# ERGO-Code/HiGHS

Hardware: AMD Instinct MI355X
Metric: PDHG iterations/sec (higher is better)
Workload: dtype f64; 1 GPU; synthetic random sparse LP 1Mx1M, 8M nnz (seed 1); m=1000000, n=1000000, nnz=7999977, parallelism=single GPU, options=presolve=off, kkt_tolerance=1e-4, adaptive step + restarts (reference defaults)

## Files before the change

### highs_amd/csrc/pdlp_halpern.cpp

```cpp
#include "pdlp_halpern.hpp"
#include "pdlp_halpernfn.hpp"

#include <algorithm>
#include <climits>
#include <cmath>
#include <cstdarg>
#include <cstdio>
#include <cstdlib>
#include <cstring>
#include <limits>

namespace pdlp {

namespace {
constexpr int kCheckInterval = 40;
constexpr int kStatSlots = 8;
constexpr int kSlotFpe = kHSlotFpe, kSlotCheck = kHSlotCheck, kSlotFpe0 = kHSlotFpe0, kSlotDiff = kHSlotDiff, kStatOut = kHStatOut;
static_assert(kSlotFpe0 == kSlotCheck + kHRowStats + kHColStats && kSlotDiff == kSlotFpe0 + 3 && kSlotDiff + 2 <= kStatOut, "stat slots");
}

double HalpernSolver::elapsed() const {
  return std::chrono::duration<double>(std::chrono::steady_clock::now() - solveBeg_).count();
}

// ... 683 lines not shown
    runBlock(false);
    enqueueFpe(kSlotFpe, nullptr);
    fetchStats(3);
    hostState_->fpe = halpernFpe(*hostState_, hostStats_ + kSlotFpe);
    put(0, hostState_->fpe);
  } else if (name == "steps") {
    const int k = out && cap > 0 ? (int)out[0] : kCheckInterval;
    if (k < 1 || k > kCheckInterval) throw std::runtime_error("steps: 1..40");
    armState();
    pushState();
    for (int i = 1; i <= k; ++i) enqueueStep(i == 1 || i == k, i);
  } else if (name == "mesh_phases") {
    double us[3] = {0, 0, 0}, cnt[3] = {0, 0, 0};
    if (mesh_) mesh_->phaseStats(us, cnt, stream_);
    for (int k = 0; k < 3; ++k) { put(k, us[k]); put(3 + k, cnt[k]); }
  } else if (name == "exchange") {
    put(0, sharded_ ? 2.0 : 0.0);
  } else if (name == "profile_on" || name == "profile_off") {
    profile_ = name == "profile_on";
  } else {
    throw std::runtime_error("unknown stage: " + name);
  }
  PDLP_HIP(hipStreamSynchronize(stream_));
}

double HalpernSolver::timeKernel(const std::string& name, int32_t reps) {
  if (reps < 1) reps = 1;
  armState();
  pushState();
  const HalpernVecs h = stepVecs(false, 2);
// ... 23 lines not shown
```

### highs_amd/csrc/pdlp_kernels.hip

```cpp
#include "pdlp_kernels.hpp"

#include <type_traits>

#include <algorithm>
#include <climits>
#include <cmath>
#include <cstddef>

#include "pdlp_checkfn.hpp"
#include "pdlp_devfn.hpp"

namespace pdlp {

namespace {

enum Epilogue { kPlain = 0, kDualStep = 1, kAtyInteract = 2, kAtyPartial = 3, kHalpernPrimal = 4, kHalpernDual = 5, kAtyFused = 6,
                kQxInteract = 7 };
constexpr bool usesDevState(int epi) {
  return epi == kDualStep || epi == kAtyInteract || epi == kAtyPartial || epi == kAtyFused || epi == kQxInteract;
}
constexpr bool isInteract(int epi) { return epi == kAtyInteract || epi == kAtyFused; }

struct SpmvArgs {
  SpmvMat A;
// ... 278 lines not shown
    }
    __syncthreads();
    for (int r = rFirst; r < r1; r += kSpmvThreads) {
      if (r != rFirst) {
        qb = a.A.beg[r] - p0;
        qe = a.A.beg[r + 1] - p0;
        pre = epi.prefetch(vecIndex(r));
      }
      const double s = majorSum(prod, qb, qe);
      epi.apply(vecIndex(r), s, pre);
    }
    epi.template finish<kSpmvThreads>(a.A.partOffset + blk, scratch);
  }
}

constexpr int kSlabSlots = 3;
template <int EPI, bool TWO, bool CC = false, bool ULO = false>
__global__ __launch_bounds__(kSlabThreads, TWO ? 2 * kSlabThreads / 256 : kSlabThreads / 256) void k_spmv_slab(const SpmvArgs a) {
  constexpr int NB = kSlabSlots;
  constexpr int GD = 1;
  constexpr bool LATE = EPI == kAtyFused && !TWO;
  if (EPI == kAtyFused && a.st->halted) {
    if (blockIdx.x == 0 && threadIdx.x < sizeof(DevState) / 4)
      reinterpret_cast<uint32_t*>(a.stOut)[threadIdx.x] = reinterpret_cast<const uint32_t*>(a.st)[threadIdx.x];
    return;
  }
  if (usesDevState(EPI) && a.st->halted) return;
  if ((EPI == kHalpernPrimal || EPI == kHalpernDual) && a.h.hs->halted) return;
  if (EPI == kPlain && !gateOpen(a.gate)) return;
  static_assert(GD >= 1 && NB >= GD + 2, "entry loads need two steps, gathers GD steps");
  const unsigned long long tProf0 = a.prof ? wall_clock64() : 0ull;
  int profBlk = (int)blockIdx.x;
// ... 80 lines not shown
      }
      for (; j < end; ++j) s += stg[j];
      wacc[lrow] = s;
    };
    if (descs == 0) {
      if (isHead) addRun();
    } else {
      const int seg = (int)__builtin_amdgcn_mbcnt_hi((uint32_t)(descs >> 32), __builtin_amdgcn_mbcnt_lo((uint32_t)descs, 0u)) + (desc ? 1 : 0);
      const int nSeg = __popcll(descs) + 1;
      for (int sg = 0; sg < nSeg; ++sg) {
        if (isHead && seg == sg) addRun();
        __builtin_amdgcn_wave_barrier();
      }
    }
  };
  const uint32_t* __restrict__ ent = a.S.ent + e0;
  const double* __restrict__ val = a.S.val + e0;
  const int cnt = e1 - e0;
  const int nG = (cnt + kWave - 1) / kWave;
  const int last = cnt > 0 ? cnt - 1 : 0;
  auto entryIndex = [&](int g) { const int q = g * kWave + lane; return q < last ? q : last; };
  auto gather = [&](uint32_t e) -> double {
    const uint32_t off = (e & mmask) << 3;
    return *reinterpret_cast<const double*>(reinterpret_cast<const char*>(in) + off);
  };
  uint32_t E[NB];
  double V[NB], X[NB];
#pragma unroll
  for (int k = 0; k < NB; ++k) {
    if (k + GD >= NB) X[(k + GD) % NB] = gather(E[(k + GD) % NB]);
    const int q = entryIndex(k);
    E[k] = ent[q];
    V[k] = val[q];
    __builtin_amdgcn_sched_barrier(0);
  }
  int nRounds = (nG + NB - 1) / NB;
  {
    int* share = reinterpret_cast<int*>(scratch);
    if (lane == 0) share[wave] = nRounds;
    __syncthreads();
#pragma unroll
    for (int w = 0; w < kWaves; ++w) nRounds = share[w] > nRounds ? share[w] : nRounds;
    __syncthreads();
  }
  for (int o = 0; o < nRounds; ++o) {
#pragma unroll
    for (int u = 0; u < NB; ++u) {
      const int g = o * NB + u;
      X[(u + GD) % NB] = gather(E[(u + GD) % NB]);
      const int nValid = cnt - g * kWave;
      const uint32_t eCur = E[u];
      const double prod = V[u] * X[u];
      {
        const int q = entryIndex(g + NB);
        E[u] = ent[q];
        V[u] = val[q];
      }
      __builtin_amdgcn_sched_barrier(0);
      consumeGroup(eCur, prod, nValid);
      if (!a.S.noPace) __syncthreads();
    }
  }
  if (a.S.noPace) __syncthreads();

  profStamp(0);
  const uint32_t* __restrict__ mask = a.S.longMask;
  auto longMajor = [&](int r) { return ((mask[r >> 5] >> (r & 31)) & 1u) != 0u; };
#pragma unroll
  for (int k = 0; k < kSlabPre; ++k) {
    const int lr = tid + k * kSlabThreads;
    if (rBase + lr < rEnd && !longMajor(rBase + lr)) epi.apply(rBase + lr, acc[lr], pre[k]);
  }
  for (int lr0 = tid + kSlabPre * kSlabThreads; rBase + lr0 < rEnd; lr0 += kSlabPre * kSlabThreads) {
    Pre more[kSlabPre];
#pragma unroll
    for (int k = 0; k < kSlabPre; ++k) {
      const int r = rBase + lr0 + k * kSlabThreads;
      more[k] = epi.prefetch(r < rEnd ? r : rEnd - 1);
// ... 495 lines not shown
    }
    return p;
  }();
  return prof;
}

template <int EPI>
void launchSpmv(const MatView& M, SpmvArgs a, hipStream_t s) {
  a.xcdMap = M.xcdMap;
  if (EPI == kDualStep && M.useSlab && M.slab.nBlocks <= 512) a.prof = slabProf();
  a.L = M.lng;
  a.A = M.csr;
  const int nTasks = M.lng.nTasks;
  if (M.useSlab && M.slab.nBlocks > 0) {
    a.S = M.slab;
    const size_t lds = (size_t)((M.slab.rowsPerBlock + 1) & ~1) * 8 + kSlabThreads * 8 + 2 * (kSlabThreads / kWave) * 8;
    const dim3 grid(M.slab.nBlocks + (nTasks + M.lng.taskGroup - 1) / M.lng.taskGroup);
    if (nTasks > 0) hipLaunchKernelGGL((k_spmv_slab<EPI, true>), grid, dim3(kSlabThreads), lds, s, a);
    else hipLaunchKernelGGL((k_spmv_slab<EPI, false>), grid, dim3(kSlabThreads), lds, s, a);
  } else if (M.csr.nBlocks > 0 || nTasks > 0) {
    const dim3 grid(M.csr.nBlocks + (nTasks + kSpmvThreads / kWave - 1) / (kSpmvThreads / kWave)), block(kSpmvThreads);
    if (M.csr.chunk == kChunkSmall) hipLaunchKernelGGL((k_spmv<EPI, kChunkSmall>), grid, block, 0, s, a);
    else hipLaunchKernelGGL((k_spmv<EPI, kChunk>), grid, block, 0, s, a);
  }
  if (nTasks > 0 && M.lng.contrib && (EPI == kDualStep || EPI == kAtyInteract || EPI == kQxInteract))
    hipLaunchKernelGGL(k_long_groups, dim3((M.lng.nSlots + kVecThreads - 1) / kVecThreads), dim3(kVecThreads), 0, s, M.lng,
                       a.st, a.part0, EPI == kAtyInteract ? a.part1 : nullptr);
}
}

void launchSpmvAxDual(const MatView& A, const IterVecs& v, const DevState* st, double* partDY, hipStream_t s) {
  SpmvArgs a{};
  a.st = st; a.v = v; a.part0 = partDY;
  launchSpmv<kDualStep>(A, a, s);
}
void launchSpmvAtyInteract(const MatView& At, const IterVecs& v, const DevState* st, double* partDX,
                           double* partInter, hipStream_t s) {
  SpmvArgs a{};
  a.st = st; a.v = v; a.part0 = partDX; a.part1 = partInter;
  launchSpmv<kAtyInteract>(At, a, s);
}
namespace {
size_t fusedLds(const MatView& At) {
  return (size_t)((At.slab.rowsPerBlock + 1) & ~1) * 8 + kSlabThreads * 8 + 2 * (kSlabThreads / kWave) * 8 + 4 * (kVecThreads / kWave) * 8 +
         sizeof(DevState) + 16;
}
}
namespace {
int fusedTaskGroups(const MatView& At) { return (At.lng.nTasks + At.lng.taskGroup - 1) / At.lng.taskGroup; }
}
int fusedCoTaskBlocks(const MatView& At, int device) {
  if (!At.useSlab || At.lng.nTasks <= 0 || At.lng.contrib != nullptr || At.slab.nBlocks <= 0) return 0;
  int perCu = 0, cus = 0;
  if (hipOccupancyMaxActiveBlocksPerMultiprocessor(&perCu, k_spmv_slab<kAtyFused, true>, kSlabThreads, fusedLds(At)) != hipSuccess) return 0;
  if (hipDeviceGetAttribute(&cus, hipDeviceAttributeMultiprocessorCount, device) != hipSuccess) return 0;
  const int groups = fusedTaskGroups(At);
  if (perCu < 2 || At.slab.nBlocks > cus || groups > cus) return 0;
  return groups;
}
int fusedAtyBlocksResident(const MatView& At, int device) {
  (void)slabProf();
  if (!At.useSlab || At.slab.nBlocks <= 0 || (At.lng.nTasks > 0 && At.lng.contrib != nullptr)) return 0;
  int perCu = 0, cus = 0;
  const hipError_t e = At.coTaskBlocks > 0
                           ? hipOccupancyMaxActiveBlocksPerMultiprocessor(&perCu, k_spmv_slab<kAtyFused, true>, kSlabThreads, fusedLds(At))
                           : hipOccupancyMaxActiveBlocksPerMultiprocessor(&perCu, k_spmv_slab<kAtyFused, false>, kSlabThreads, fusedLds(At));
  if (e != hipSuccess) return 0;
  if (hipDeviceGetAttribute(&cus, hipDeviceAttributeMultiprocessorCount, device) != hipSuccess) return 0;
  return perCu * cus;
}
int fusedAtyBlocks(const MatView& At) { return At.slab.nBlocks + At.coTaskBlocks; }
void launchSpmvAtyFusedPrimal(const MatView& At, const IterVecs& v, const DevState* stIn, DevState* stOut,
                              const double* partDY, int32_t nDY, double* partDX, double* partInter, unsigned long long* bar,
                              hipStream_t s, int32_t timeoutMs, int32_t faultTrial) {
  SpmvArgs a{};
  a.barLimit = (unsigned long long)(timeoutMs > 0 ? timeoutMs : 1000) * 100000ull;
  a.faultTrial = faultTrial;
  a.coTaskBlocks = At.lng.nTasks > 0 ? At.coTaskBlocks : 0;
  a.inlineTasks = At.lng.nTasks > 0 && a.coTaskBlocks == 0 ? 1 : 0;
  a.touchTail = At.touchTail;
  a.st = stIn; a.v = v; a.part0 = partDX; a.part1 = partInter;
  a.stOut = stOut; a.partDY = partDY; a.nDY = nDY; a.nDX = At.nPartials; a.bar = bar;
  if (At.slab.nBlocks <= 512) a.prof = slabProf();
  a.xcdMap = At.xcdMap; a.L = At.lng; a.A = At.csr; a.S = At.slab;
  const dim3 gridTwo(At.slab.nBlocks + a.coTaskBlocks), gridOne(At.slab.nBlocks), block(kSlabThreads);
  const size_t lds = fusedLds(At);
  auto launchTwo = [&](auto cc, auto ulo) {
    hipLaunchKernelGGL((k_spmv_slab<kAtyFused, true, decltype(cc)::value, decltype(ulo)::value>), gridTwo, block, lds, s, a);
  };
  auto launchOne = [&](auto cc, auto ulo) {
    hipLaunchKernelGGL((k_spmv_slab<kAtyFused, false, decltype(cc)::value, decltype(ulo)::value>), gridOne, block, lds, s, a);
  };
  auto pick = [&](auto&& launch) {
    using T = std::true_type; using F = std::false_type;
    if (v.constCached) { if (v.lowerUniform) launch(T{}, T{}); else launch(T{}, F{}); }
    else { if (v.lowerUniform) launch(F{}, T{}); else launch(F{}, F{}); }
  };
  if (a.coTaskBlocks > 0) pick(launchTwo);
  else pick(launchOne);
}
void launchSpmvAtyPartial(const MatView& At, const IterVecs& v, const DevState* st, double* out, hipStream_t s) {
  SpmvArgs a{};
  a.st = st; a.v = v; a.out = out;
  launchSpmv<kAtyPartial>(At, a, s);
}
void launchHalpernPrimal(const MatView& At, const HalpernVecs& h, hipStream_t s) {
// ... 184 lines not shown
```

### highs_amd/csrc/pdlp_kernels.hpp

```cpp
#pragma once
#include <hip/hip_runtime.h>

#include <cstdint>

#include "pdlp_env.hpp"

namespace pdlp {

constexpr int kChunk = 2048;
constexpr int kChunkSmall = 512;
constexpr int64_t kChunkSmallBelowNnz = 1 << 18;
inline int32_t spmvChunkFor(int64_t nnz) { return nnz < kChunkSmallBelowNnz ? kChunkSmall : kChunk; }
constexpr int kSpmvThreads = 256;
constexpr int kMaxMajorsPerBlock = 2048;
constexpr int kVecThreads = 256;

struct DevState {
  double eta;
  double beta;
  double tau, sigma;
  double primalStep, dualStep;
  double sumPrimalStep, sumDualStep;
  double avgW;
  double avgWx;
// ... 79 lines not shown
  int32_t nSlots;
  int32_t groupSize;
  int32_t taskGroup;
};

constexpr int kSlabThreads = 1024;
constexpr int kSlabMaxRows = 16384;
struct SlabMat {
  const int32_t* wavePtr;
  const uint32_t* ent;
  const double* val;
  const uint32_t* longMask;
  const int32_t* waveBeg;
  int32_t nMajor, nBlocks, rowsPerBlock, minorBits;
  int32_t noPace;
};
constexpr int kSlabTileLog2 = 14;

struct MatView {
  SpmvMat csr;
  SlabMat slab;
  LongMat lng;
  int32_t useSlab;
  int32_t nPartials;
  int32_t xcdMap;
  int32_t coTaskBlocks;
  int32_t touchTail;
};

struct IterVecs {
  double* x[2];
// ... 205 lines not shown
```

### highs_amd/csrc/pdlp_setup.hip

```cpp
#include "pdlp_setup.hpp"

#include <cstring>

#include <rocprim/rocprim.hpp>

#include <algorithm>
#include <cmath>
#include <limits>

namespace pdlp {

namespace {

constexpr int kT = 256;
inline int gridFor(int64_t n) { return (int)std::max<int64_t>(1, std::min<int64_t>((n + kT - 1) / kT, 65535 * 16)); }
#define GSTRIDE(i, n) for (int64_t i = (int64_t)blockIdx.x * blockDim.x + threadIdx.x; i < (n); i += (int64_t)gridDim.x * blockDim.x)

constexpr double kBoundInf = 1e20;

__device__ __forceinline__ bool isEqKind(int k) { return k == kRowEq || k == kRowBound || k == kRowFree; }
__global__ void k_row_classify(const double* __restrict__ lo, const double* __restrict__ up, int m, double infThresh,
                               int freeKind, int32_t* kind, int32_t* eqFlag, int32_t* ineqFlag, int32_t* slackFlag) {
  GSTRIDE(i, m) {
    const bool hl = lo[i] > -infThresh, hu = up[i] < infThresh;
// ... 677 lines not shown
  sortByKey(keys.get(), nnz, (uint64_t)keyMax, sortedKeys, perm, s);
  L.wavePtr.alloc((size_t)nWaves + 1);
  hipLaunchKernelGGL(k_wave_ptr, dim3(gridFor(nWaves + 1)), dim3(kT), 0, s, sortedKeys.get(), nnz, nWaves, S,
                     L.wavePtr.get());
  L.nnzShort = fetchOne(L.wavePtr.get() + nWaves, s);
  L.ent.alloc((size_t)L.nnzShort + 1);
  L.val.alloc((size_t)L.nnzShort + 1);
  L.ent.zero(s);
  L.val.zero(s);
  if (L.nnzShort > 0)
    hipLaunchKernelGGL(k_slab_entries, dim3(gridFor(L.nnzShort)), dim3(kT), 0, s, perm.get(), M.major.get(),
                       M.idx.get(), M.val.get(), L.nnzShort, waveOf.get(), L.waveBeg.get(), L.minorBits, L.ent.get(), L.val.get());
  PDLP_HIP(hipStreamSynchronize(s));
}

}
```

### highs_amd/csrc/pdlp_setup.hpp

```cpp
#pragma once
#include <hip/hip_runtime.h>

#include <cstdint>
#include <vector>

#include "pdlp_device.hpp"
#include "pdlp_host.hpp"
#include "pdlp_kernels.hpp"

namespace pdlp {

struct DeviceCsrData {
  DeviceArray<int32_t> beg, idx, major;
  DeviceArray<double> val;
  int32_t nMajor = 0, nMinor = 0;
  int64_t nnz = 0;
};

struct MatrixKeep {
  int64_t nnz0 = 0;
  DeviceArray<int32_t> aStart, aIndex;
  DeviceArray<int32_t> cscBeg, cscIdx, cscCol;
  DeviceArray<int32_t> aBeg, aMajor, aIdx;
  DeviceArray<int32_t> permA;
// ... 60 lines not shown
struct DeviceSlabLayout {
  int32_t rowsPerBlock = 0, nBlocks = 0, minorBits = 0, nLong = 0;
  int64_t nnzShort = 0;
  std::vector<int32_t> hostWaveBeg;
  DeviceArray<int32_t> wavePtr, waveBeg;
  DeviceArray<uint32_t> ent, longMask;
  DeviceArray<double> val;
  DeviceCsrData longCsr;
  DeviceArray<int32_t> longMap;
  std::vector<int32_t> hostLongBeg;
};
void gpuSlabPartition(const DeviceCsrData& M, int32_t longLimit, int32_t majorCost, hipStream_t s, DeviceSlabLayout& out);
void gpuBuildSlabLayout(const DeviceCsrData& M, int32_t longLimit, int32_t slabWidthLog2, int32_t majorCost, hipStream_t s,
                        DeviceSlabLayout& out);

}
```

### highs_amd/csrc/pdlp_solver.cpp

```cpp
#include "pdlp_solver.hpp"
#include "pdlp_detmath.h"
#include "pdlp_update.hpp"

#include <algorithm>
#include <climits>
#include <cmath>
#include <cstdarg>
#include <cstdio>
#include <cstdlib>
#include <cstring>

namespace pdlp {

namespace {
constexpr int kStatRowCur = 0, kStatRowAvg = kRowStats, kStatColCur = 2 * kRowStats,
              kStatColAvg = 2 * kRowStats + kColStats, kStatTotal = 2 * kRowStats + 2 * kColStats;
constexpr int kGraphTrials = 42;
constexpr int kGraphMinTodo = 30;
constexpr int kCheckInterval = kReleaseInterval;
}

namespace {
constexpr int32_t kSlabLongLimit = 256;
constexpr int32_t kSlabAutoMinor = 1 << 18;
// ... 219 lines not shown
      for (int r = 0; r < 3; ++r) launchSpmvPlain(M.view(), in, out, s);
      PDLP_HIP(hipEventRecord(e1, s));
      PDLP_HIP(hipEventSynchronize(e1));
      float ms = 0.f;
      PDLP_HIP(hipEventElapsedTime(&ms, e0, e1));
      if (first || ms < 0.97f * best) { best = ms; bestMap = M.xcdMap; bestFree = M.noPace; first = false; }
    }
  }
  M.xcdMap = bestMap;
  M.noPace = bestFree;
  (void)hipEventDestroy(e0);
  (void)hipEventDestroy(e1);
  return best / 3.f;
}

void buildSlabTuned(DeviceMatrix& out, DeviceCsrData& M, const DevSwitches& sw, hipStream_t s) {
  out.buildFromDevice(M, sw, s);
  if (!out.useSlab || sw.slabW > 0 || sw.slabTune == 0 || M.nnz < ((int64_t)1 << 20)) return;
  if (out.estRunLen < 2.0) return;
  DeviceArray<double> in, res;
  in.alloc((size_t)std::max(M.nMinor, 1));
  res.alloc((size_t)std::max(M.nMajor, 1));
  in.zero(s);
  float best = tuneXcdMap(out, sw, in.get(), res.get(), s);
  out.mapTuned = true;
  const int32_t autoW = out.slabWidthLog2;
  for (int32_t W : {13, 11}) {
    if (W == autoW || ((int64_t)1 << W) >= (int64_t)M.nMinor) continue;
    DevSwitches sw2 = sw;
    sw2.slabW = W;
    DeviceMatrix cand;
    cand.majorCost = out.majorCost;
    cand.balanceTaskBlocks = out.balanceTaskBlocks;
    cand.buildFromDevice(M, sw2, s);
    const float t = tuneXcdMap(cand, sw, in.get(), res.get(), s);
    cand.mapTuned = true;
    if (t < 0.97f * best) {
      best = t;
      out = std::move(cand);
    }
    PDLP_HIP(hipStreamSynchronize(s));
  }
}

DevSwitches DevSwitches::fromEnv() {
  DevSwitches w;
  auto num = [](const char* name, int dflt) {
    const char* e = getenv(name);
    return e ? atoi(e) : dflt;
  };
  auto dev = [](const char* name, int dflt) {
    const char* e = devEnv(name);
    return e ? atoi(e) : dflt;
  };
  w.gpuSetup = num("PDLP_MI355X_GPU_SETUP", -1);
  w.fused = num("PDLP_MI355X_FUSED", -1);
  w.persistent = num("PDLP_MI355X_PERSISTENT", -1);
  w.persistentQp = num("PDLP_MI355X_PERSISTENT_QP", -1);
  w.barrierTimeoutMs = num("PDLP_MI355X_BARRIER_TIMEOUT_MS", 1000);
  {
    const char* e = getenv("PDLP_MI355X_EXCHANGE");
    w.exchange = e ? e : "";
  }
  w.graph = dev("PDLP_MI355X_GRAPH", -1);
  w.forceComm = dev("PDLP_MI355X_FORCE_COMM", 0);
  w.slab = dev("PDLP_MI355X_SLAB", -1);
  w.slabW = dev("PDLP_MI355X_SLAB_W", 0);
  w.xcdMap = dev("PDLP_MI355X_XCD_MAP", -1);
  w.slabPace = dev("PDLP_MI355X_SLAB_PACE", -1);
  w.slabTune = dev("PDLP_MI355X_SLAB_TUNE", 1);
  w.fusedCoTasks = dev("PDLP_MI355X_FUSED_COTASKS", -1);
  w.constCached = dev("PDLP_MI355X_CONST_CACHED", -1);
  w.touchTail = dev("PDLP_MI355X_TOUCH_TAIL", 1);
  w.xcdLocal = dev("PDLP_MI355X_XCD_LOCAL", -1);
  w.hierBarrier = dev("PDLP_MI355X_HIER_BARRIER", -1);
  w.deviceCheck = dev("PDLP_MI355X_DEVICE_CHECK", -1);
  w.checkSmall = dev("PDLP_MI355X_CHECK_SMALL", -1);
  w.primalInA = dev("PDLP_MI355X_PRIMAL_IN_A", -1);
  w.fault = dev("PDLP_MI355X_FAULT", 0);
  if (w.fault) fprintf(stderr, "pdlp_mi355x: PDLP_MI355X_FAULT=%d is set — a TEST hook that makes a barrier launch time out on purpose; "
                               "this solve will stall for the barrier timeout and continue on the slower plain-launch path\n", w.fault);
  return w;
}

Solver::DeviceGate& Solver::deviceGate(int device) {
// ... 1777 lines not shown
    put(1, (double)nPass_);
    put(2, (double)vecs_.lowerUniform);
    put(3, graphExec_ ? 1.0 : 0.0);
    put(4, (double)(mk_.bytes() + sizeof(int32_t) * (srcAVal_.size() + srcASlab_.size() + srcAtVal_.size() + srcAtSlab_.size()) +
                    sizeof(double) * updMat_.size()));
    put(5, matrixUpdatable_ ? 1.0 : 0.0);
    put(6, (double)(hk_.bytes() + sizeof(int32_t) * (srcQVal_.size() + srcQSlab_.size()) + sizeof(double) * updQ_.size()));
    put(7, hessianUpdatable_ ? 1.0 : 0.0);
  } else if (name == "update_values_seconds") {
    for (int k = 0; k < 4; ++k) put(k, updHessSeconds_[k]);
    put(4, (double)updRecaptured_);
    put(5, setupSeconds_);
  } else if (name == "update_matrix_seconds") {
    for (int k = 0; k < 8; ++k) put(k, updMatSeconds_[k]);
    put(8, setupSeconds_);
  } else if (name == "trial_launches") {
    const int fw = meshMode_ ? mesh_->args().fusedWait : 0;
    const double qx = sharded_ && hasQoff_ ? 1.0 : 0.0;
    put(0, meshMode_ ? 9.0 - 2.0 * fw + qx : sharded_ ? 7.0 + qx : persistent_ ? 0.0 : fused_ ? 2.0 : 3.0);
  } else if (name == "trial_barriers") {
    put(0, !persistent_ ? 0.0 : primalInA_ ? 2.0 : 3.0);
  } else if (name == "check_launches") {
    put(0, !devCheck_ ? 0.0 : sharded_ ? (mesh_ && mesh_->args().fusedWait == 2 ? 14.0 : 26.0) + (hasQoff_ ? 1.0 : 0.0) : persistent_ && checkSmall_ ? 1.0 : 10.0);
  } else if (name == "small_loop") {
    put(0, persistent_ ? (double)smallGrid_ : 0.0);
    put(1, persistent_ ? (double)smallMode() : -1.0);
    put(2, persistent_ && checkSmall_ ? 1.0 : 0.0);
  } else if (name == "barrier_fallbacks") {
    put(0, (double)barrierFallbacks_);
  } else if (name == "persistent_launches") {
// ... 82 lines not shown
```

### highs_amd/csrc/pdlp_solver.hpp

```cpp
#pragma once
#include <hip/hip_runtime.h>

#include <chrono>
#include <cstdint>
#include <map>
#include <mutex>
#include <stdexcept>
#include <string>
#include <vector>

#include "pdlp_device.hpp"
#include "pdlp_host.hpp"
#include "pdlp_kernels.hpp"
#include "pdlp_mesh.hpp"
#include "pdlp_round.hpp"
#include "pdlp_setup.hpp"

namespace pdlp {

struct DevSwitches {
  int graph = -1, forceComm = 0, gpuSetup = -1;
  int slab = -1;
  int slabW = 0;
  int xcdMap = -1, slabPace = -1;
  int slabTune = 1;
  int fusedCoTasks = -1;
  int touchTail = 1;
  int constCached = -1;
  int fused = -1, persistent = -1, xcdLocal = -1, hierBarrier = -1, deviceCheck = -1, checkSmall = -1;
  int persistentQp = -1;
  int primalInA = -1;
  int barrierTimeoutMs = 1000;
  int fault = 0;
  std::string exchange;
  static DevSwitches fromEnv();
};

struct DeviceMatrix {
  DeviceArray<int32_t> beg, idx, blockBeg, wavePtr, waveBeg;
  DeviceArray<uint32_t> ent, longMask;
  DeviceArray<double> val, slabVal;
  DeviceArray<LongTask> lTasks;
  DeviceArray<double> lSegSum, lContrib;
  DeviceArray<uint32_t> lTicket;
  int32_t nLong = 0, nTasks = 0, longSlots = 0, longGroup = 1, taskGroup = 4;
  bool balanceTaskBlocks = true;
  int32_t majorCost = kSlabMajorCostRows;
  int32_t fusedCoTasks = 0;
  int32_t touchTail = 1;
  int32_t nMajor = 0, nBlocks = 0;
  int32_t chunk = kChunk;
  int64_t nnz = 0;
  bool useSlab = false;
  int32_t noPace = 0;
  int32_t slabWidthLog2 = 0;
  double estRunLen = 1.0;
  bool mapTuned = false;
  int32_t xcdMap = 1;
  SlabMat slab{};
  void upload(const Compressed& c, int32_t nMajor_, int32_t nMinor_, const DevSwitches& sw, hipStream_t s);
  void buildFromDevice(DeviceCsrData& M, const DevSwitches& sw, hipStream_t s);
  MatView view() const;
  int32_t nPartials() const { return (useSlab ? slab.nBlocks : 0) + nBlocks + longSlots; }

 private:
  void uploadPlans(const std::vector<int32_t>& hostBeg, int32_t nCsrMajor, const int32_t* longVecIndex, hipStream_t s,
                   const int32_t* hostLongIdx = nullptr, const std::vector<int8_t>* tileOwner = nullptr, int32_t tileLog2 = 0);
  static bool touchesFewTiles(const std::vector<int32_t>& lo, const std::vector<int32_t>& hi, const std::vector<int32_t>& cnt);
};

float tuneXcdMap(DeviceMatrix& M, const DevSwitches& sw, const double* in, double* out, hipStream_t s);
void buildSlabTuned(DeviceMatrix& out, DeviceCsrData& M, const DevSwitches& sw, hipStream_t s);

class Comm;
// ... 281 lines not shown
```

Measured before the change: 7704 it/s.

## Add gather-ordered slab SpMV layout with per-slab LDS chunk buffers and autotuned selection

Adds a gather-order variant of the slab SpMV. Entries are regrouped by slab so that products are written into double-buffered LDS chunk buffers indexed by slot, then reduced per row using packed 4-bit counts and a DPP wave prefix sum. Setup kernels build the new layout. At build time the tuner times it against the existing layout and keeps it only if it is clearly faster. The aim is better gather locality and less per-group segmented reduction, at the cost of more LDS, which may lower occupancy, plus extra setup work and code complexity.

After: 8029 it/s (median of 5 runs). 4.2% higher.

```diff
diff --git a/highs_amd/csrc/pdlp_halpern.cpp b/highs_amd/csrc/pdlp_halpern.cpp
--- a/highs_amd/csrc/pdlp_halpern.cpp
+++ b/highs_amd/csrc/pdlp_halpern.cpp
@@ -721,6 +721,10 @@
     double us[3] = {0, 0, 0}, cnt[3] = {0, 0, 0};
     if (mesh_) mesh_->phaseStats(us, cnt, stream_);
     for (int k = 0; k < 3; ++k) { put(k, us[k]); put(3 + k, cnt[k]); }
+  } else if (name == "slab_gather_order") {
+    put(0, dA_.useSlab && dA_.slab.gord ? 1.0 : 0.0); put(1, (double)dA_.gordWhy);
+    put(2, dAt_.useSlab && dAt_.slab.gord ? 1.0 : 0.0); put(3, (double)dAt_.gordWhy);
+    put(4, 0.0); put(5, (double)kGordNotTried);
   } else if (name == "exchange") {
     put(0, sharded_ ? 2.0 : 0.0);
   } else if (name == "profile_on" || name == "profile_off") {
diff --git a/highs_amd/csrc/pdlp_kernels.hip b/highs_amd/csrc/pdlp_kernels.hip
--- a/highs_amd/csrc/pdlp_kernels.hip
+++ b/highs_amd/csrc/pdlp_kernels.hip
@@ -316,8 +316,17 @@
   }
 }
 
+__device__ __forceinline__ int waveInclusiveSum(int v) {
+  v += __builtin_amdgcn_update_dpp(0, v, 0x111, 0xf, 0xf, false);
+  v += __builtin_amdgcn_update_dpp(0, v, 0x112, 0xf, 0xf, false);
+  v += __builtin_amdgcn_update_dpp(0, v, 0x114, 0xf, 0xf, false);
+  v += __builtin_amdgcn_update_dpp(0, v, 0x118, 0xf, 0xf, false);
+  v += __builtin_amdgcn_update_dpp(0, v, 0x142, 0xa, 0xf, false);
+  v += __builtin_amdgcn_update_dpp(0, v, 0x143, 0xc, 0xf, false);
+  return v;
+}
 constexpr int kSlabSlots = 3;
-template <int EPI, bool TWO, bool CC = false, bool ULO = false>
+template <int EPI, bool TWO, bool CC = false, bool ULO = false, bool GORD = false>
 __global__ __launch_bounds__(kSlabThreads, TWO ? 2 * kSlabThreads / 256 : kSlabThreads / 256) void k_spmv_slab(const SpmvArgs a) {
   constexpr int NB = kSlabSlots;
   constexpr int GD = 1;
@@ -428,54 +437,145 @@
       }
     }
   };
-  const uint32_t* __restrict__ ent = a.S.ent + e0;
-  const double* __restrict__ val = a.S.val + e0;
-  const int cnt = e1 - e0;
-  const int nG = (cnt + kWave - 1) / kWave;
-  const int last = cnt > 0 ? cnt - 1 : 0;
-  auto entryIndex = [&](int g) { const int q = g * kWave + lane; return q < last ? q : last; };
-  auto gather = [&](uint32_t e) -> double {
-    const uint32_t off = (e & mmask) << 3;
-    return *reinterpret_cast<const double*>(reinterpret_cast<const char*>(in) + off);
-  };
-  uint32_t E[NB];
-  double V[NB], X[NB];
-#pragma unroll
-  for (int k = 0; k < NB; ++k) {
-    if (k + GD >= NB) X[(k + GD) % NB] = gather(E[(k + GD) % NB]);
-    const int q = entryIndex(k);
-    E[k] = ent[q];
-    V[k] = val[q];
-    __builtin_amdgcn_sched_barrier(0);
-  }
-  int nRounds = (nG + NB - 1) / NB;
-  {
-    int* share = reinterpret_cast<int*>(scratch);
-    if (lane == 0) share[wave] = nRounds;
+  if constexpr (!GORD) {
+    const uint32_t* __restrict__ ent = a.S.ent + e0;
+    const double* __restrict__ val = a.S.val + e0;
+    const int cnt = e1 - e0;
+    const int nG = (cnt + kWave - 1) / kWave;
+    const int last = cnt > 0 ? cnt - 1 : 0;
+    auto entryIndex = [&](int g) { const int q = g * kWave + lane; return q < last ? q : last; };
+    auto gather = [&](uint32_t e) -> double {
+      const uint32_t off = (e & mmask) << 3;
+      return *reinterpret_cast<const double*>(reinterpret_cast<const char*>(in) + off);
+    };
+    uint32_t E[NB];
+    double V[NB], X[NB];
+  #pragma unroll
+    for (int k = 0; k < NB; ++k) {
+      if (k + GD >= NB) X[(k + GD) % NB] = gather(E[(k + GD) % NB]);
+      const int q = entryIndex(k);
+      E[k] = ent[q];
+      V[k] = val[q];
+      __builtin_amdgcn_sched_barrier(0);
+    }
+    int nRounds = (nG + NB - 1) / NB;
+    {
+      int* share = reinterpret_cast<int*>(scratch);
+      if (lane == 0) share[wave] = nRounds;
+      __syncthreads();
+  #pragma unroll
+      for (int w = 0; w < kWaves; ++w) nRounds = share[w] > nRounds ? share[w] : nRounds;
+      __syncthreads();
+    }
+    for (int o = 0; o < nRounds; ++o) {
+  #pragma unroll
+      for (int u = 0; u < NB; ++u) {
+        const int g = o * NB + u;
+        X[(u + GD) % NB] = gather(E[(u + GD) % NB]);
+        const int nValid = cnt - g * kWave;
+        const uint32_t eCur = E[u];
+        const double prod = V[u] * X[u];
+        {
+          const int q = entryIndex(g + NB);
+          E[u] = ent[q];
+          V[u] = val[q];
+        }
+        __builtin_amdgcn_sched_barrier(0);
+        consumeGroup(eCur, prod, nValid);
+        if (!a.S.noPace) __syncthreads();
+      }
+    }
+    if (a.S.noPace) __syncthreads();
+  } else {
+    const int W = a.S.widthLog2, nS = a.S.nSlabs, cap = a.S.chunkCap, cw = a.S.cntWords;
+    const uint32_t lmask = (1u << W) - 1u;
+    double* pbuf = reinterpret_cast<double*>(smem + a.S.gordOff);
+    uint32_t* cntL = reinterpret_cast<uint32_t*>(pbuf + 2 * cap);
+    {
+      const uint32_t* __restrict__ src = a.S.cnt4 + (size_t)blk * nS * cw;
+      for (int i = tid; i < nS * cw; i += kSlabThreads) cntL[i] = src[i];
+    }
+    const int g0 = e0, nG = e1 - e0;
+    const uint32_t* __restrict__ ent = a.S.ent + (size_t)g0 * kWave;
+    const double* __restrict__ val = a.S.val + (size_t)g0 * kWave;
+    const int32_t* __restrict__ gEnd = a.S.grpEnd + (size_t)gw * (nS + 1);
+    const int32_t* __restrict__ sBase = a.S.slotBase + (size_t)gw * nS;
+    const int lastG = nG > 0 ? nG - 1 : 0;
+    auto entryIndex = [&](int g) { return (g < lastG ? g : lastG) * kWave + lane; };
+    int sq = 0, sqEnd = ldUniform(gEnd + 1);
+    auto gather = [&](uint32_t e, int gq) -> double {
+      while (gq < nG && gq >= sqEnd) { ++sq; sqEnd = ldUniform(gEnd + sq + 1); }
+      const uint32_t off = (((uint32_t)sq << W) + (e & lmask)) << 3;
+      return *reinterpret_cast<const double*>(reinterpret_cast<const char*>(in) + off);
+    };
+    const int wOff = wBeg - rBase;
+    const int addPerStep = nG > 0 ? (((Rw + kWave - 1) / kWave) * nS + nG - 1) / nG : 1;
+    int ps = -1, pk = 0, pfirst = 0;
+    auto addRound = [&]() {
+      const double* __restrict__ pb = pbuf + (ps & 1) * cap;
+      const uint32_t* __restrict__ cs = cntL + ps * cw;
+      const int k0 = pk * kWave;
+      const int lr = wOff + k0 + lane;
+      const int c = k0 + lane < Rw ? (int)((cs[lr >> 3] >> ((lr & 7) * 4)) & 15u) : 0;
+      const int incl = waveInclusiveSum(c);
+      if (c) {
+        const double* __restrict__ q = pb + pfirst + incl - c;
+        const double t0 = q[0], t1 = q[1], t2 = q[2], t3 = q[3];
+        double sum = acc[lr];
+        sum += t0;
+        if (c > 1) sum += t1;
+        if (c > 2) sum += t2;
+        if (c > 3) sum += t3;
+        for (int j = 4; j < c; ++j) sum += q[j];
+        acc[lr] = sum;
+      }
+      pfirst += __builtin_amdgcn_readlane(incl, kWave - 1);
+      ++pk;
+      if (pk * kWave >= Rw) ps = -1;
+    };
+    auto flush = [&](int sl) {
+      while (ps >= 0) addRound();
+      __syncthreads();
+      if (Rw > 0) { ps = sl; pk = 0; pfirst = ldUniform(sBase + sl); }
+    };
+    uint32_t E[NB];
+    double V[NB], X[NB];
+#pragma unroll
+    for (int k = 0; k < NB; ++k) {
+      if (k + GD >= NB) X[(k + GD) % NB] = gather(E[(k + GD) % NB], k + GD - NB);
+      const int q = entryIndex(k);
+      E[k] = ent[q];
+      V[k] = val[q];
+      __builtin_amdgcn_sched_barrier(0);
+    }
+    int sc = 0, scEnd = ldUniform(gEnd + 1);
+    const int nRounds = (nG + NB - 1) / NB;
+    for (int o = 0; o < nRounds; ++o) {
+#pragma unroll
+      for (int u = 0; u < NB; ++u) {
+        const int g = o * NB + u;
+        X[(u + GD) % NB] = gather(E[(u + GD) % NB], g + GD);
+        const uint32_t eCur = E[u];
+        const double prod = V[u] * X[u];
+        {
+          const int q = entryIndex(g + NB);
+          E[u] = ent[q];
+          V[u] = val[q];
+        }
+        __builtin_amdgcn_sched_barrier(0);
+        while (sc < nS && g >= scEnd) {
+          flush(sc);
+          ++sc;
+          scEnd = sc < nS ? ldUniform(gEnd + sc + 1) : 0x7fffffff;
+        }
+        if (g < nG) pbuf[(sc & 1) * cap + (eCur >> W)] = prod;
+        for (int t = 0; t < addPerStep && ps >= 0; ++t) addRound();
+      }
+    }
+    for (; sc < nS; ++sc) flush(sc);
+    while (ps >= 0) addRound();
     __syncthreads();
-#pragma unroll
-    for (int w = 0; w < kWaves; ++w) nRounds = share[w] > nRounds ? share[w] : nRounds;
-    __syncthreads();
-  }
-  for (int o = 0; o < nRounds; ++o) {
-#pragma unroll
-    for (int u = 0; u < NB; ++u) {
-      const int g = o * NB + u;
-      X[(u + GD) % NB] = gather(E[(u + GD) % NB]);
-      const int nValid = cnt - g * kWave;
-      const uint32_t eCur = E[u];
-      const double prod = V[u] * X[u];
-      {
-        const int q = entryIndex(g + NB);
-        E[u] = ent[q];
-        V[u] = val[q];
-      }
-      __builtin_amdgcn_sched_barrier(0);
-      consumeGroup(eCur, prod, nValid);
-      if (!a.S.noPace) __syncthreads();
-    }
-  }
-  if (a.S.noPace) __syncthreads();
+  }
 
   profStamp(0);
   const uint32_t* __restrict__ mask = a.S.longMask;
@@ -1001,9 +1101,14 @@
   const int nTasks = M.lng.nTasks;
   if (M.useSlab && M.slab.nBlocks > 0) {
     a.S = M.slab;
-    const size_t lds = (size_t)((M.slab.rowsPerBlock + 1) & ~1) * 8 + kSlabThreads * 8 + 2 * (kSlabThreads / kWave) * 8;
+    const size_t ldsBase = (size_t)((M.slab.rowsPerBlock + 1) & ~1) * 8 + kSlabThreads * 8 + 2 * (kSlabThreads / kWave) * 8;
+    a.S.gordOff = (int32_t)ldsBase;
+    const size_t lds = ldsBase + slabGatherOrderLds(M.slab);
     const dim3 grid(M.slab.nBlocks + (nTasks + M.lng.taskGroup - 1) / M.lng.taskGroup);
-    if (nTasks > 0) hipLaunchKernelGGL((k_spmv_slab<EPI, true>), grid, dim3(kSlabThreads), lds, s, a);
+    if (M.slab.gord) {
+      if (nTasks > 0) hipLaunchKernelGGL((k_spmv_slab<EPI, true, false, false, true>), grid, dim3(kSlabThreads), lds, s, a);
+      else hipLaunchKernelGGL((k_spmv_slab<EPI, false, false, false, true>), grid, dim3(kSlabThreads), lds, s, a);
+    } else if (nTasks > 0) hipLaunchKernelGGL((k_spmv_slab<EPI, true>), grid, dim3(kSlabThreads), lds, s, a);
     else hipLaunchKernelGGL((k_spmv_slab<EPI, false>), grid, dim3(kSlabThreads), lds, s, a);
   } else if (M.csr.nBlocks > 0 || nTasks > 0) {
     const dim3 grid(M.csr.nBlocks + (nTasks + kSpmvThreads / kWave - 1) / (kSpmvThreads / kWave)), block(kSpmvThreads);
@@ -1027,10 +1132,19 @@
   a.st = st; a.v = v; a.part0 = partDX; a.part1 = partInter;
   launchSpmv<kAtyInteract>(At, a, s);
 }
+size_t slabFusedLdsBase(int32_t rowsPerBlock) {
+  return ((size_t)((rowsPerBlock + 1) & ~1) * 8 + kSlabThreads * 8 + 2 * (kSlabThreads / kWave) * 8 + 4 * (kVecThreads / kWave) * 8 +
+          sizeof(DevState) + 16 + 15) & ~(size_t)15;
+}
 namespace {
-size_t fusedLds(const MatView& At) {
-  return (size_t)((At.slab.rowsPerBlock + 1) & ~1) * 8 + kSlabThreads * 8 + 2 * (kSlabThreads / kWave) * 8 + 4 * (kVecThreads / kWave) * 8 +
-         sizeof(DevState) + 16;
+size_t fusedLdsBase(const MatView& At) { return slabFusedLdsBase(At.slab.rowsPerBlock); }
+size_t fusedLds(const MatView& At) { return fusedLdsBase(At) + slabGatherOrderLds(At.slab); }
+hipError_t fusedOccupancy(int* perCu, const MatView& At, bool two) {
+  if (At.slab.gord)
+    return two ? hipOccupancyMaxActiveBlocksPerMultiprocessor(perCu, k_spmv_slab<kAtyFused, true, false, false, true>, kSlabThreads, fusedLds(At))
+               : hipOccupancyMaxActiveBlocksPerMultiprocessor(perCu, k_spmv_slab<kAtyFused, false, false, false, true>, kSlabThreads, fusedLds(At));
+  return two ? hipOccupancyMaxActiveBlocksPerMultiprocessor(perCu, k_spmv_slab<kAtyFused, true>, kSlabThreads, fusedLds(At))
+             : hipOccupancyMaxActiveBlocksPerMultiprocessor(perCu, k_spmv_slab<kAtyFused, false>, kSlabThreads, fusedLds(At));
 }
 }
 namespace {
@@ -1039,7 +1153,7 @@
 int fusedCoTaskBlocks(const MatView& At, int device) {
   if (!At.useSlab || At.lng.nTasks <= 0 || At.lng.contrib != nullptr || At.slab.nBlocks <= 0) return 0;
   int perCu = 0, cus = 0;
-  if (hipOccupancyMaxActiveBlocksPerMultiprocessor(&perCu, k_spmv_slab<kAtyFused, true>, kSlabThreads, fusedLds(At)) != hipSuccess) return 0;
+  if (fusedOccupancy(&perCu, At, true) != hipSuccess) return 0;
   if (hipDeviceGetAttribute(&cus, hipDeviceAttributeMultiprocessorCount, device) != hipSuccess) return 0;
   const int groups = fusedTaskGroups(At);
   if (perCu < 2 || At.slab.nBlocks > cus || groups > cus) return 0;
@@ -1049,9 +1163,7 @@
   (void)slabProf();
   if (!At.useSlab || At.slab.nBlocks <= 0 || (At.lng.nTasks > 0 && At.lng.contrib != nullptr)) return 0;
   int perCu = 0, cus = 0;
-  const hipError_t e = At.coTaskBlocks > 0
-                           ? hipOccupancyMaxActiveBlocksPerMultiprocessor(&perCu, k_spmv_slab<kAtyFused, true>, kSlabThreads, fusedLds(At))
-                           : hipOccupancyMaxActiveBlocksPerMultiprocessor(&perCu, k_spmv_slab<kAtyFused, false>, kSlabThreads, fusedLds(At));
+  const hipError_t e = fusedOccupancy(&perCu, At, At.coTaskBlocks > 0);
   if (e != hipSuccess) return 0;
   if (hipDeviceGetAttribute(&cus, hipDeviceAttributeMultiprocessorCount, device) != hipSuccess) return 0;
   return perCu * cus;
@@ -1072,11 +1184,14 @@
   a.xcdMap = At.xcdMap; a.L = At.lng; a.A = At.csr; a.S = At.slab;
   const dim3 gridTwo(At.slab.nBlocks + a.coTaskBlocks), gridOne(At.slab.nBlocks), block(kSlabThreads);
   const size_t lds = fusedLds(At);
+  a.S.gordOff = (int32_t)fusedLdsBase(At);
   auto launchTwo = [&](auto cc, auto ulo) {
-    hipLaunchKernelGGL((k_spmv_slab<kAtyFused, true, decltype(cc)::value, decltype(ulo)::value>), gridTwo, block, lds, s, a);
+    if (At.slab.gord) hipLaunchKernelGGL((k_spmv_slab<kAtyFused, true, decltype(cc)::value, decltype(ulo)::value, true>), gridTwo, block, lds, s, a);
+    else hipLaunchKernelGGL((k_spmv_slab<kAtyFused, true, decltype(cc)::value, decltype(ulo)::value>), gridTwo, block, lds, s, a);
   };
   auto launchOne = [&](auto cc, auto ulo) {
-    hipLaunchKernelGGL((k_spmv_slab<kAtyFused, false, decltype(cc)::value, decltype(ulo)::value>), gridOne, block, lds, s, a);
+    if (At.slab.gord) hipLaunchKernelGGL((k_spmv_slab<kAtyFused, false, decltype(cc)::value, decltype(ulo)::value, true>), gridOne, block, lds, s, a);
+    else hipLaunchKernelGGL((k_spmv_slab<kAtyFused, false, decltype(cc)::value, decltype(ulo)::value>), gridOne, block, lds, s, a);
   };
   auto pick = [&](auto&& launch) {
     using T = std::true_type; using F = std::false_type;
diff --git a/highs_amd/csrc/pdlp_kernels.hpp b/highs_amd/csrc/pdlp_kernels.hpp
--- a/highs_amd/csrc/pdlp_kernels.hpp
+++ b/highs_amd/csrc/pdlp_kernels.hpp
@@ -117,7 +117,20 @@
   const int32_t* waveBeg;
   int32_t nMajor, nBlocks, rowsPerBlock, minorBits;
   int32_t noPace;
-};
+  int32_t gord;
+  int32_t widthLog2, nSlabs;
+  int32_t chunkCap;
+  int32_t cntWords;
+  int32_t gordOff;
+  const int32_t* grpEnd;
+  const int32_t* slotBase;
+  const uint32_t* cnt4;
+};
+inline size_t slabGatherOrderLds(const SlabMat& S) {
+  return S.gord ? (size_t)2 * S.chunkCap * 8 + (size_t)S.nSlabs * S.cntWords * 4 : 0;
+}
+constexpr int64_t kSlabLdsBytes = 160 * 1024;
+size_t slabFusedLdsBase(int32_t rowsPerBlock);
 constexpr int kSlabTileLog2 = 14;
 
 struct MatView {
diff --git a/highs_amd/csrc/pdlp_setup.hip b/highs_amd/csrc/pdlp_setup.hip
--- a/highs_amd/csrc/pdlp_setup.hip
+++ b/highs_amd/csrc/pdlp_setup.hip
@@ -715,4 +715,177 @@
   PDLP_HIP(hipStreamSynchronize(s));
 }
 
-}
+namespace {
+__global__ void k_gord_seg(const int32_t* __restrict__ wavePtr, const uint32_t* __restrict__ ent, int nWaves, int S, int W,
+                           uint32_t mmask, int32_t* segBeg) {
+  GSTRIDE(t, (int64_t)nWaves * (S + 1)) {
+    const int gw = (int)(t / (S + 1)), sl = (int)(t % (S + 1));
+    int lo = wavePtr[gw], hi = wavePtr[gw + 1];
+    while (lo < hi) {
+      const int mid = (lo + hi) >> 1;
+      if ((int)((ent[mid] & mmask) >> W) < sl) lo = mid + 1; else hi = mid;
+    }
+    segBeg[t] = lo;
+  }
+}
+__host__ __device__ inline int gordGroupsOf(int nGroups, int w, int sl) {
+  const int j0 = (w - sl % kSlabWavesPerBlock + kSlabWavesPerBlock) % kSlabWavesPerBlock;
+  return nGroups > j0 ? (nGroups - j0 + kSlabWavesPerBlock - 1) / kSlabWavesPerBlock : 0;
+}
+__global__ void k_gord_meta(const int32_t* __restrict__ segBeg, int nWaves, int S, int32_t* grpEnd, int32_t* slotBase,
+                            int32_t* waveGroups, int32_t* maxChunk) {
+  GSTRIDE(gw, nWaves) {
+    const int b = (int)gw / kSlabWavesPerBlock, w = (int)gw % kSlabWavesPerBlock;
+    int run = 0, big = 0;
+    for (int sl = 0; sl < S; ++sl) {
+      int n = 0, base = 0;
+      for (int v = 0; v < kSlabWavesPerBlock; ++v) {
+        const int32_t* q = segBeg + (size_t)(b * kSlabWavesPerBlock + v) * (S + 1) + sl;
+        if (v == w) base = n;
+        n += q[1] - q[0];
+      }
+      grpEnd[(size_t)gw * (S + 1) + sl] = run;
+      slotBase[(size_t)gw * S + sl] = base;
+      run += gordGroupsOf((n + 63) / 64, w, sl);
+      big = n > big ? n : big;
+    }
+    grpEnd[(size_t)gw * (S + 1) + S] = run;
+    waveGroups[gw] = run;
+    if (w == 0) atomicMax(maxChunk, big);
+  }
+}
+__global__ void k_gord_counts(const int32_t* __restrict__ wavePtr, const int32_t* __restrict__ waveBeg,
+                              const uint32_t* __restrict__ ent, int64_t nShort, int nWaves, int S, int W, int mb, int cw,
+                              uint32_t* cnt4, int32_t* tooMany) {
+  const uint32_t mmask = (1u << mb) - 1u;
+  GSTRIDE(q, nShort) {
+    int lo = 0, hi = nWaves;
+    while (hi - lo > 1) {
+      const int mid = (lo + hi) >> 1;
+      if (wavePtr[mid] <= (int)q) lo = mid; else hi = mid;
+    }
+    const int gw = lo;
+    auto key = [&](int64_t i) { const uint32_t e = ent[i]; return ((uint64_t)((e & mmask) >> W) << 32) | (e >> mb); };
+    const uint64_t k = key(q);
+    if (q > wavePtr[gw] && key(q - 1) == k) continue;
+    const int end = wavePtr[gw + 1];
+    int c = 1;
+    while (c < 16 && q + c < end && key(q + c) == k) ++c;
+    if (c > 15) { *tooMany = 1; continue; }
+    const int b = gw / kSlabWavesPerBlock;
+    const int lr = waveBeg[gw] - waveBeg[b * kSlabWavesPerBlock] + (int)(uint32_t)k;
+    atomicOr(cnt4 + ((size_t)b * S + (size_t)(k >> 32)) * cw + (lr >> 3), (uint32_t)c << ((lr & 7) * 4));
+  }
+}
+constexpr int kGordFillThreads = 1024;
+__global__ __launch_bounds__(kGordFillThreads) void k_gord_fill(const int32_t* __restrict__ segBeg, const uint32_t* __restrict__ ent,
+                                                                const double* __restrict__ val, const int32_t* __restrict__ grpPtr,
+                                                                const int32_t* __restrict__ grpEnd, int S, int W, int mb, int P,
+                                                                int slotBits, uint32_t dumpSlot, uint32_t* gEnt, double* gVal) {
+  extern __shared__ uint32_t keys[];
+  __shared__ int segB[kSlabWavesPerBlock], sBase[kSlabWavesPerBlock + 1];
+  const int b = blockIdx.x / S, sl = blockIdx.x % S, tid = threadIdx.x;
+  if (tid == 0) {
+    int n = 0;
+    for (int v = 0; v < kSlabWavesPerBlock; ++v) {
+      const int32_t* q = segBeg + (size_t)(b * kSlabWavesPerBlock + v) * (S + 1) + sl;
+      segB[v] = q[0];
+      sBase[v] = n;
+      n += q[1] - q[0];
+    }
+    sBase[kSlabWavesPerBlock] = n;
+  }
+  __syncthreads();
+  const int n = sBase[kSlabWavesPerBlock];
+  if (n == 0) return;
+  const uint32_t lmask = (uint32_t)((1ull << W) - 1ull), mmask = (uint32_t)((1ull << mb) - 1ull);
+  auto source = [&](int slot) {
+    int v = 0;
+    while (sBase[v + 1] <= slot) ++v;
+    return segB[v] + (slot - sBase[v]);
+  };
+  for (int i = tid; i < P; i += kGordFillThreads)
+    keys[i] = i < n ? ((ent[source(i)] & mmask & lmask) << slotBits) | (uint32_t)i : 0xffffffffu;
+  __syncthreads();
+  for (int k = 2; k <= P; k <<= 1) {
+    for (int j = k >> 1; j > 0; j >>= 1) {
+      for (int i = tid; i < P; i += kGordFillThreads) {
+        const int x = i ^ j;
+        if (x > i) {
+          const uint32_t ka = keys[i], kb = keys[x];
+          if (((i & k) == 0) == (ka > kb)) { keys[i] = kb; keys[x] = ka; }
+        }
+      }
+      __syncthreads();
+    }
+  }
+  const int nOut = (n + 63) / 64 * 64;
+  const uint32_t lastMinor = keys[n - 1] >> slotBits;
+  for (int i = tid; i < nOut; i += kGordFillThreads) {
+    const int j = i >> 6, w = (j + sl) % kSlabWavesPerBlock, gw = b * kSlabWavesPerBlock + w;
+    const size_t dst = ((size_t)grpPtr[gw] + grpEnd[(size_t)gw * (S + 1) + sl] + j / kSlabWavesPerBlock) * 64 + (i & 63);
+    if (i < n) {
+      const uint32_t k = keys[i], slot = k & ((1u << slotBits) - 1u);
+      gEnt[dst] = (slot << W) | (k >> slotBits);
+      gVal[dst] = val[source((int)slot)];
+    } else {
+      gEnt[dst] = (dumpSlot << W) | lastMinor;
+      gVal[dst] = 0.0;
+    }
+  }
+}
+}
+
+bool gpuSlabGatherOrder(const GatherOrderSource& in, int64_t ldsBudget, hipStream_t s, GatherOrderLayout& L) {
+  const int32_t nWaves = in.nBlocks * kSlabWavesPerBlock;
+  const int32_t W = in.widthLog2, mb = in.minorBits;
+  if (W <= 0) throw std::runtime_error("slab gather order: the layout has no slab width");
+  const int32_t S = std::max(1, (int32_t)(((int64_t)in.nMinor + ((int64_t)1 << W) - 1) >> W));
+  L = GatherOrderLayout{};
+  L.nSlabs = S;
+  L.cntWords = (in.rowsPerBlock + 7) / 8;
+  if ((int64_t)nWaves * (S + 1) >= (int64_t)0x7fffffff) { L.refused = kGordTooManySlabs; return false; }
+  if ((int64_t)S * L.cntWords * 4 > ldsBudget) { L.refused = kGordLds; return false; }
+  DeviceArray<int32_t> segBeg, waveGroups, flags;
+  segBeg.alloc((size_t)nWaves * (S + 1));
+  waveGroups.alloc((size_t)nWaves + 1);
+  flags.alloc(2);
+  waveGroups.zero(s);
+  flags.zero(s);
+  L.grpPtr.alloc((size_t)nWaves + 1);
+  L.grpEnd.alloc((size_t)nWaves * (S + 1));
+  L.slotBase.alloc((size_t)nWaves * S);
+  L.cnt4.alloc((size_t)in.nBlocks * S * L.cntWords);
+  L.cnt4.zero(s);
+  const uint32_t mmask = (uint32_t)((1ull << mb) - 1ull);
+  hipLaunchKernelGGL(k_gord_seg, dim3(gridFor((int64_t)nWaves * (S + 1))), dim3(kT), 0, s, in.wavePtr, in.ent, nWaves, S, W, mmask,
+                     segBeg.get());
+  hipLaunchKernelGGL(k_gord_meta, dim3(gridFor(nWaves)), dim3(kT), 0, s, segBeg.get(), nWaves, S, L.grpEnd.get(), L.slotBase.get(),
+                     waveGroups.get(), flags.get());
+  if (in.nnzShort > 0)
+    hipLaunchKernelGGL(k_gord_counts, dim3(gridFor(in.nnzShort)), dim3(kT), 0, s, in.wavePtr, in.waveBeg, in.ent, in.nnzShort, nWaves,
+                       S, W, mb, L.cntWords, L.cnt4.get(), flags.get() + 1);
+  exclusiveSum(waveGroups.get(), L.grpPtr.get(), (int64_t)nWaves + 1, s);
+  int32_t hf[2] = {0, 0};
+  flags.download(hf, 2, s);
+  const int64_t nGroups = fetchOne(L.grpPtr.get() + nWaves, s);
+  if (hf[1]) { L.refused = kGordCount; return false; }
+  const int32_t maxChunk = hf[0];
+  L.chunkCap = (maxChunk + 2) & ~1;
+  int P = 64, slotBits = 6;
+  while (P < maxChunk) { P <<= 1; ++slotBits; }
+  if (W + slotBits > 32 || (int64_t)L.chunkCap > ((int64_t)1 << (32 - W)) || (size_t)P * 4 > 60 * 1024) { L.refused = kGordSlotField; return false; }
+  if ((int64_t)2 * L.chunkCap * 8 + (int64_t)S * L.cntWords * 4 > ldsBudget) { L.refused = kGordLds; return false; }
+  L.nGroups = nGroups;
+  L.ent.alloc((size_t)(nGroups + 1) * 64);
+  L.val.alloc((size_t)(nGroups + 1) * 64);
+  L.ent.zero(s);
+  L.val.zero(s);
+  hipLaunchKernelGGL(k_gord_fill, dim3(in.nBlocks * S), dim3(kGordFillThreads), (size_t)P * 4, s, segBeg.get(), in.ent, in.val,
+                     L.grpPtr.get(), L.grpEnd.get(), S, W, mb, P, slotBits, (uint32_t)(L.chunkCap - 1), L.ent.get(), L.val.get());
+  PDLP_HIP(hipGetLastError());
+  PDLP_HIP(hipStreamSynchronize(s));
+  return true;
+}
+
+}
diff --git a/highs_amd/csrc/pdlp_setup.hpp b/highs_amd/csrc/pdlp_setup.hpp
--- a/highs_amd/csrc/pdlp_setup.hpp
+++ b/highs_amd/csrc/pdlp_setup.hpp
@@ -98,4 +98,29 @@
 void gpuBuildSlabLayout(const DeviceCsrData& M, int32_t longLimit, int32_t slabWidthLog2, int32_t majorCost, hipStream_t s,
                         DeviceSlabLayout& out);
 
+struct GatherOrderSource {
+  const int32_t* wavePtr;
+  const uint32_t* ent;
+  const double* val;
+  const int32_t* waveBeg;
+  int64_t nnzShort;
+  int32_t nBlocks, rowsPerBlock, minorBits, widthLog2, nMinor;
+};
+enum GatherOrderRefusal : int32_t {
+  kGordOk = 0,
+  kGordCount = 4,
+  kGordSlotField = 5,
+  kGordLds = 6,
+  kGordTooManySlabs = 8,
+};
+struct GatherOrderLayout {
+  DeviceArray<int32_t> grpPtr, grpEnd, slotBase;
+  DeviceArray<uint32_t> ent, cnt4;
+  DeviceArray<double> val;
+  int64_t nGroups = 0;
+  int32_t nSlabs = 0, chunkCap = 0, cntWords = 0;
+  int32_t refused = kGordOk;
+};
+bool gpuSlabGatherOrder(const GatherOrderSource& in, int64_t ldsBudget, hipStream_t s, GatherOrderLayout& out);
+
 }
diff --git a/highs_amd/csrc/pdlp_solver.cpp b/highs_amd/csrc/pdlp_solver.cpp
--- a/highs_amd/csrc/pdlp_solver.cpp
+++ b/highs_amd/csrc/pdlp_solver.cpp
@@ -257,33 +257,101 @@
   return best / 3.f;
 }
 
+namespace {
+void swapGatherOrder(DeviceMatrix& out, GatherOrderLayout& L, bool in) {
+  std::swap(out.wavePtr, L.grpPtr);
+  std::swap(out.ent, L.ent);
+  std::swap(out.slabVal, L.val);
+  std::swap(out.grpEnd, L.grpEnd);
+  std::swap(out.slotBase, L.slotBase);
+  std::swap(out.cnt4, L.cnt4);
+  out.slab.wavePtr = out.wavePtr.get();
+  out.slab.ent = out.ent.get();
+  out.slab.val = out.slabVal.get();
+  out.slab.gord = in ? 1 : 0;
+  out.slab.widthLog2 = out.slabWidthLog2;
+  out.slab.nSlabs = L.nSlabs;
+  out.slab.chunkCap = L.chunkCap;
+  out.slab.cntWords = L.cntWords;
+  out.slab.grpEnd = out.grpEnd.get();
+  out.slab.slotBase = out.slotBase.get();
+  out.slab.cnt4 = out.cnt4.get();
+}
+int32_t buildGatherOrder(DeviceMatrix& out, int32_t nMinor, hipStream_t s, GatherOrderLayout& L) {
+  GatherOrderSource src{out.wavePtr.get(), out.ent.get(), out.slabVal.get(), out.waveBeg.get(), (int64_t)out.ent.size() - 1,
+                        out.slab.nBlocks, out.slab.rowsPerBlock, out.slab.minorBits, out.slabWidthLog2, nMinor};
+  const int64_t budget = (out.nTasks > 0 ? kSlabLdsBytes / 2 : kSlabLdsBytes) - (int64_t)slabFusedLdsBase(out.slab.rowsPerBlock);
+  if (!gpuSlabGatherOrder(src, budget, s, L)) return L.refused;
+  swapGatherOrder(out, L, true);
+  return kGordOk;
+}
+}
+
 void buildSlabTuned(DeviceMatrix& out, DeviceCsrData& M, const DevSwitches& sw, hipStream_t s) {
   out.buildFromDevice(M, sw, s);
-  if (!out.useSlab || sw.slabW > 0 || sw.slabTune == 0 || M.nnz < ((int64_t)1 << 20)) return;
-  if (out.estRunLen < 2.0) return;
+  out.gordWhy = sw.slabGord == 0 ? kGordSwitchedOff : kGordNotTried;
+  if (!out.useSlab) return;
+  const bool forced = sw.slabGord == 1;
+  const bool tune = !(sw.slabW > 0 || sw.slabTune == 0 || M.nnz < ((int64_t)1 << 20));
+  if (!tune && !forced) return;
   DeviceArray<double> in, res;
-  in.alloc((size_t)std::max(M.nMinor, 1));
-  res.alloc((size_t)std::max(M.nMajor, 1));
-  in.zero(s);
-  float best = tuneXcdMap(out, sw, in.get(), res.get(), s);
+  float best = 0.f;
+  if (tune) {
+    in.alloc((size_t)std::max(M.nMinor, 1));
+    res.alloc((size_t)std::max(M.nMajor, 1));
+    in.zero(s);
+  }
+  if (tune && out.estRunLen >= 2.0) {
+    best = tuneXcdMap(out, sw, in.get(), res.get(), s);
+    out.mapTuned = true;
+    const int32_t autoW = out.slabWidthLog2;
+    for (int32_t W : {13, 11}) {
+      if (W == autoW || ((int64_t)1 << W) >= (int64_t)M.nMinor) continue;
+      DevSwitches sw2 = sw;
+      sw2.slabW = W;
+      DeviceMatrix cand;
+      cand.majorCost = out.majorCost;
+      cand.balanceTaskBlocks = out.balanceTaskBlocks;
+      cand.buildFromDevice(M, sw2, s);
+      const float t = tuneXcdMap(cand, sw, in.get(), res.get(), s);
+      cand.mapTuned = true;
+      if (t < 0.97f * best) {
+        best = t;
+        out = std::move(cand);
+      }
+      PDLP_HIP(hipStreamSynchronize(s));
+    }
+    out.gordWhy = sw.slabGord == 0 ? kGordSwitchedOff : kGordLongRuns;
+    if (!forced) return;
+  }
+  if (sw.slabGord == 0) return;
+  GatherOrderLayout L;
+  const int32_t refused = buildGatherOrder(out, M.nMinor, s, L);
+  if (refused != kGordOk) {
+    out.gordWhy = refused;
+    if (forced) fprintf(stderr, "pdlp_mi355x: PDLP_MI355X_SLAB_GORD=1, but the gather-order arrangement was refused (reason %d: %s); "
+                                "the operand stays on the slab layout as it is\n", refused,
+                        refused == kGordCount ? "a major with more than 15 entries in one slab"
+                        : refused == kGordSlotField ? "a chunk exceeds the slot field"
+                        : refused == kGordLds ? "the chunk buffers do not fit the block's LDS" : "too many slabs");
+    return;
+  }
+  out.gordWhy = kGordInUse;
+  if (forced) return;
+  const int32_t map1 = out.xcdMap, pace1 = out.noPace;
+  swapGatherOrder(out, L, false);
+  best = tuneXcdMap(out, sw, in.get(), res.get(), s);
+  const int32_t map0 = out.xcdMap, pace0 = out.noPace;
+  out.xcdMap = map1; out.noPace = pace1;
+  swapGatherOrder(out, L, true);
+  const float t = tuneXcdMap(out, sw, in.get(), res.get(), s);
+  if (!(t < 0.97f * best)) {
+    swapGatherOrder(out, L, false);
+    out.xcdMap = map0; out.noPace = pace0;
+    out.gordWhy = kGordNotFaster;
+  }
   out.mapTuned = true;
-  const int32_t autoW = out.slabWidthLog2;
-  for (int32_t W : {13, 11}) {
-    if (W == autoW || ((int64_t)1 << W) >= (int64_t)M.nMinor) continue;
-    DevSwitches sw2 = sw;
-    sw2.slabW = W;
-    DeviceMatrix cand;
-    cand.majorCost = out.majorCost;
-    cand.balanceTaskBlocks = out.balanceTaskBlocks;
-    cand.buildFromDevice(M, sw2, s);
-    const float t = tuneXcdMap(cand, sw, in.get(), res.get(), s);
-    cand.mapTuned = true;
-    if (t < 0.97f * best) {
-      best = t;
-      out = std::move(cand);
-    }
-    PDLP_HIP(hipStreamSynchronize(s));
-  }
+  PDLP_HIP(hipStreamSynchronize(s));
 }
 
 DevSwitches DevSwitches::fromEnv() {
@@ -312,6 +380,7 @@
   w.xcdMap = dev("PDLP_MI355X_XCD_MAP", -1);
   w.slabPace = dev("PDLP_MI355X_SLAB_PACE", -1);
   w.slabTune = dev("PDLP_MI355X_SLAB_TUNE", 1);
+  w.slabGord = dev("PDLP_MI355X_SLAB_GORD", -1);
   w.fusedCoTasks = dev("PDLP_MI355X_FUSED_COTASKS", -1);
   w.constCached = dev("PDLP_MI355X_CONST_CACHED", -1);
   w.touchTail = dev("PDLP_MI355X_TOUCH_TAIL", 1);
@@ -2119,6 +2188,12 @@
   } else if (name == "update_matrix_seconds") {
     for (int k = 0; k < 8; ++k) put(k, updMatSeconds_[k]);
     put(8, setupSeconds_);
+  } else if (name == "slab_gather_order") {
+    const DeviceMatrix* ops[3] = {&dA_, &dAt_, &dQ_};
+    for (int k = 0; k < 3; ++k) {
+      put(2 * k, ops[k]->useSlab && ops[k]->slab.gord ? 1.0 : 0.0);
+      put(2 * k + 1, (double)ops[k]->gordWhy);
+    }
   } else if (name == "trial_launches") {
     const int fw = meshMode_ ? mesh_->args().fusedWait : 0;
     const double qx = sharded_ && hasQoff_ ? 1.0 : 0.0;
diff --git a/highs_amd/csrc/pdlp_solver.hpp b/highs_amd/csrc/pdlp_solver.hpp
--- a/highs_amd/csrc/pdlp_solver.hpp
+++ b/highs_amd/csrc/pdlp_solver.hpp
@@ -25,6 +25,7 @@
   int xcdMap = -1, slabPace = -1;
   int slabTune = 1;
   int fusedCoTasks = -1;
+  int slabGord = -1;
   int touchTail = 1;
   int constCached = -1;
   int fused = -1, persistent = -1, xcdLocal = -1, hierBarrier = -1, deviceCheck = -1, checkSmall = -1;
@@ -34,6 +35,14 @@
   int fault = 0;
   std::string exchange;
   static DevSwitches fromEnv();
+};
+
+enum : int32_t {
+  kGordInUse = 0,
+  kGordLongRuns = 1,
+  kGordNotTried = 2,
+  kGordSwitchedOff = 3,
+  kGordNotFaster = 7,
 };
 
 struct DeviceMatrix {
@@ -58,6 +67,9 @@
   bool mapTuned = false;
   int32_t xcdMap = 1;
   SlabMat slab{};
+  DeviceArray<int32_t> grpEnd, slotBase;
+  DeviceArray<uint32_t> cnt4;
+  int32_t gordWhy = kGordNotTried;
   void upload(const Compressed& c, int32_t nMajor_, int32_t nMinor_, const DevSwitches& sw, hipStream_t s);
   void buildFromDevice(DeviceCsrData& M, const DevSwitches& sw, hipStream_t s);
   MatView view() const;
```
